# qway/nerfmeshes

Measured on NVIDIA H100. Metric: rays/sec, higher is better.
Workload: dtype f16x3 split operands, f32 accumulate

## Files before the change

include/nerfmeshes_b200.h:

```cpp
#ifndef NERFMESHES_B200_H
#define NERFMESHES_B200_H

#include <stdint.h>

#ifdef __cplusplus
extern "C" {
#endif

#define NM_VERSION 100

typedef struct NmNetDesc {
  int32_t num_layers;
  int32_t hidden_size;
  int32_t skip_step;
  int32_t num_encoding_fn_xyz;
  int32_t num_encoding_fn_dir;
  int32_t include_input_xyz;
  int32_t include_input_dir;
  int32_t log_sampling_xyz;
  int32_t log_sampling_dir;
  int32_t use_viewdirs;
} NmNetDesc;

enum {
// ... 170 lines not shown
int nm_debug_gemm(NmHandle h, const float* a_dev, const float* b_dev, int M, int N, int K, int n_passes, float* d_dev,
                  void* stream);

int nm_debug_mlp_backward(NmHandle h, int which, const float* pts_dev, const float* dirs_dev, int64_t M, const float* dout_dev,
                          void* stream);

int nm_debug_composite_backward(NmHandle h, const float* raw_dev, const float* t_dev, const float* dirs_dev,
                                const float* d_rgb_dev, int64_t R, int S, float noise_std, uint64_t seed, int white_bg,
                                float* dout_dev, void* stream);
int nm_debug_composite(NmHandle h, const float* raw_dev, const float* t_dev, const float* dirs_dev, int64_t R, int S,
                       float noise_std, uint64_t seed, int white_bg, int training, float thr, const NmRenderOut* out_dev,
                       void* stream);
int nm_debug_sample_pdf(NmHandle h, const float* t_c_dev, const float* w_c_dev, const float* u_dev, int64_t R, int Nc, int Nf,
                        int perturb, uint64_t seed, float* t_out_dev, void* stream);

int nm_debug_pack(const NmNetDesc* desc, int n_tensors, const char* const* names, const float* const* tensors_host,
                  const int64_t* numel, int sigma_only, void* program_out, size_t program_cap, uint8_t* pack_out,
                  size_t pack_cap, size_t* pack_need);
int nm_debug_pack_wide(const NmNetDesc* desc, int n_tensors, const char* const* names, const float* const* tensors_host,
                       const int64_t* numel, int sigma_only, void* program_out, size_t program_cap, uint8_t* pack_out,
                       size_t pack_cap, size_t* pack_need);

int nm_debug_tile_schedule(int samples_per_ray, int64_t n_tiles, int grid, int cta, int64_t* tiles_out, int64_t cap, int64_t* n_out);

int nm_kernel_flags(NmHandle h, int32_t* out2);
int nm_check_flags(NmHandle h, void* stream);

int64_t nm_launch_count(NmHandle h);
int nm_set_timing(NmHandle h, int enable);
double nm_mlp_time_ms(NmHandle h, int64_t* points_out, int64_t* launches_out);

#ifdef __cplusplus
}
#endif
#endif
```

nerfmeshes_b200/_lib.py:

```python
import ctypes as C
import os

_HERE = os.path.dirname(os.path.abspath(__file__))
LIB_PATH = os.path.join(_HERE, "lib", "libnerfmeshes_b200.so")


class NmNetDesc(C.Structure):
    _fields_ = [(n, C.c_int32) for n in (
        "num_layers", "hidden_size", "skip_step", "num_encoding_fn_xyz", "num_encoding_fn_dir",
        "include_input_xyz", "include_input_dir", "log_sampling_xyz", "log_sampling_dir", "use_viewdirs")]


class NmRenderCfg(C.Structure):
    _fields_ = [("num_coarse", C.c_int32), ("num_fine", C.c_int32), ("lindisp", C.c_int32), ("perturb", C.c_int32),
                ("white_background", C.c_int32), ("noise_std", C.c_float), ("attenuation_threshold", C.c_float),
                ("precision", C.c_int32), ("act_scale_log2", C.c_int32)]


OUT_FIELDS = ("rgb", "depth", "depth_raw", "acc", "disp", "weights", "mask_weights", "t_vals",
              "coarse_rgb", "coarse_acc", "coarse_disp", "coarse_weights")


class NmRenderOut(C.Structure):
    _fields_ = [(n, C.c_void_p) for n in OUT_FIELDS]
# ... 53 lines not shown
    "nm_query_host": (C.c_int, [_P, _P, _I, _P, _L, _P, _I, C.c_uint64, C.POINTER(NmRenderOut)]),
    "nm_render_image_host": (C.c_int, [_P, _P, _I, _I, _D, _I, _I, _I, _P, _I, C.c_uint64, C.POINTER(NmRenderOut)]),
    "nm_point_mlp_host": (C.c_int, [_P, _I, _P, _P, _L, _P, _I]),
    "nm_zero_grad": (C.c_int, [_P, _P]),
    "nm_backward_rays": (C.c_int, [_P, _P, _I, _P, _L, _P, _P, _P, _I, C.c_uint64, _P, _P, _P]),
    "nm_loss_backward": (C.c_int, [_P, _P, _I, _P, _L, _P, _P, _P, _I, C.c_uint64, _P, _P, _P]),
    "nm_get_grad": (C.c_int, [_P, _I, C.c_char_p, _P, _L, _P]),
    "nm_ray_voxel_indices": (C.c_int, [_P, _P, _I, _P, _L, _P, _P, _P, _P]),
    "nm_ray_voxel_indices_ex": (C.c_int, [_P, _P, _I, _P, _L, _P, _I, C.c_uint64, _P, _P, _P]),
    "nm_tree_integrate": (C.c_int, [_P, _P, _P, _P, _L, _P, C.c_int32, C.c_int32, _P]),
    "nm_debug_gemm": (C.c_int, [_P, _P, _P, _I, _I, _I, _I, _P, _P]),
    "nm_debug_mlp_backward": (C.c_int, [_P, _I, _P, _P, _L, _P, _P]),
    "nm_debug_composite_backward": (C.c_int, [_P, _P, _P, _P, _P, _L, _I, _F, C.c_uint64, _I, _P, _P]),
    "nm_debug_composite": (C.c_int, [_P, _P, _P, _P, _L, _I, _F, C.c_uint64, _I, _I, _F, C.POINTER(NmRenderOut), _P]),
    "nm_debug_sample_pdf": (C.c_int, [_P, _P, _P, _P, _L, _I, _I, _I, C.c_uint64, _P, _P]),
    "nm_debug_pack": (C.c_int, [C.POINTER(NmNetDesc), _I, C.POINTER(C.c_char_p), C.POINTER(_P), C.POINTER(C.c_int64), _I, _P,
                               C.c_size_t, _P, C.c_size_t, C.POINTER(C.c_size_t)]),
    "nm_debug_pack_wide": (C.c_int, [C.POINTER(NmNetDesc), _I, C.POINTER(C.c_char_p), C.POINTER(_P), C.POINTER(C.c_int64), _I,
                                    _P, C.c_size_t, _P, C.c_size_t, C.POINTER(C.c_size_t)]),
    "nm_kernel_flags": (C.c_int, [_P, C.POINTER(C.c_int32)]),
    "nm_check_flags": (C.c_int, [_P, _P]),
    "nm_ndc_rays": (C.c_int, [_P, _I, _I, _D, _D, _P, _I, _P, _L, _P, _P, _P]),
    "nm_launch_count": (C.c_int64, [_P]),
    "nm_debug_tile_schedule": (C.c_int, [_I, _L, _I, _I, _P, _L, _P]),
    "nm_set_timing": (C.c_int, [_P, _I]),
    "nm_mlp_time_ms": (C.c_double, [_P, C.POINTER(C.c_int64), C.POINTER(C.c_int64)]),
}

_lib = None


class NmError(RuntimeError):
    pass


def load():
    global _lib
    if _lib is not None:
        return _lib
    if not os.path.exists(LIB_PATH):
        raise NmError(f"{LIB_PATH} is missing: build it with `python -m nerfmeshes_b200.build` "
                      "(there is no fallback implementation)")
    lib = C.CDLL(LIB_PATH)
    for name, (res, args) in _SIGNATURES.items():
        fn = getattr(lib, name)
        fn.restype = res
        fn.argtypes = args
# ... 12 lines not shown
```

nerfmeshes_b200/csrc/nm_api.cu:

```cuda
#include <cmath>
#include <cstdio>
#include <cstdlib>
#include <algorithm>
#include <cstring>
#include <vector>

#include "nm_common.h"
#include "nm_gemm.h"

namespace nm {
const char* last_error();
}

using namespace nm;

namespace {

struct Buf {
  void* p = nullptr;
  size_t cap = 0;
  int ensure(size_t bytes) {
    if (bytes <= cap) return 0;
    if (p) cudaFree(p);
    p = nullptr; cap = 0;
// ... 9 lines not shown

}

struct NmHandle_t {
  int device = 0;
  int num_sms = 0;
  NmRenderCfg cfg{};
  NetDev nets[2];
  bool has_fine = false;
  NmNetDesc desc[2]{};
  Buf s_table, u_table, voxels;
  int V = 0;
  Buf t_c, raw_c, w_c, t_f, raw_f, t_u, dirs, origins, lin[3], small, stage_in[3], stage_out[12];
  int lin_n[3] = {0, 0, 0};
  int* d_err = nullptr;
  int* h_err = nullptr;
  double* d_stats = nullptr;
  cudaStream_t own_stream = nullptr;
  int64_t launches = 0;
  bool timing = false;
  std::vector<cudaEvent_t> ev;
  size_t ev_used = 0;
  int64_t mlp_points = 0, mlp_launches = 0;
  Buf mc_ws, mc_ws2;
  int64_t mc_counts[2] = {0, 0};
  Buf ss_tab, ss_ws;
  Buf ms_ws, nn_ws;
  Buf cc_ws;
  Buf dc_ws;
  Buf tx_ws;
  Buf rs_ws;
  Buf sf_ws;
  Buf sp_ws;
  int sp_grid[4] = {0, 0, 0, 0};
  const float* sp_vol = nullptr;
  struct OccGrid {
    bool valid = false;
    bool stale = false;
    float lo[3], hi[3], inv[3];
    int G = 0;
    Buf bits;
  } occ[2];
  Buf oc_ws;
  Buf sk_ws;
  Buf ts_ws[2], ts_pts[2];
  Buf train_ws_c;
// ... 95 lines not shown
  }
  return 0;
}

int run_mlp(NmHandle h, int which, bool sigma_only, const MlpInput& in, float* out, cudaStream_t st, const MlpEmit* emit = nullptr,
            const CompositeArgs* comp = nullptr) {
  const NetDev& net = h->nets[which];
  NM_CHECK(net.loaded, "weights of network %d not loaded", which);
  cudaEvent_t e0 = nullptr, e1 = nullptr;
  if (h->timing) {
    while (h->ev.size() < h->ev_used + 2) {
      cudaEvent_t e;
      NM_CUDA(cudaEventCreate(&e));
      h->ev.push_back(e);
    }
    e0 = h->ev[h->ev_used++]; e1 = h->ev[h->ev_used++];
    NM_CUDA(cudaEventRecord(e0, st));
  }
  int rc;
  if (h->cfg.precision == NM_PREC_FP32) rc = launch_mlp_simt(net, sigma_only, in, out, st, &h->launches);
  else rc = launch_mlp_tc(net, sigma_only, h->cfg.precision == NM_PREC_FAST ? 1 : 3, h->cfg.act_scale_log2, in, out,
                          h->num_sms, h->d_err, st, &h->launches, emit, comp);
  if (rc) return rc;
  if (h->timing) {
    NM_CUDA(cudaEventRecord(e1, st));
    h->mlp_points += in.M;
    h->mlp_launches += 1;
  }
  return 0;
}

constexpr uint64_t kNoiseSaltMain = 0x5bd1e995ull, kNoiseSaltCoarse = 0x7f4a7c15a3c59ac3ull;
constexpr uint64_t kVoxelSalt = 0xd1b54a32d192ed03ull, kInvCdfSalt = 0x9e3779b9ull;

struct RayBatch {
  const float* origins; int o_stride; const float* dirs; long long R;
  float nf[2]; const float* near_dev; const float* far_dev;
};

float* off(float* p, long long n) { return p ? p + n : nullptr; }

struct TrainSkip {
  bool emit = false;
  double budget = 0;
  double* committed = nullptr;
  long long M = 0;
// ... 95 lines not shown
    for (long long j0 = 0; j0 < M; j0 += P) {
      const long long m = (M - j0 < P) ? M - j0 : P;
      if (!ts)
        if (int e = launch_occ_stage(idx + j0, m, s, rb.origins, rb.o_stride, rb.dirs, t, pts, dirs, st, &h->launches)) return e;
      MlpInput in{};
      in.mode = IN_POINTS; in.pts = ts ? pts + 3 * j0 : pts; in.dirs = ts ? dirs + 3 * j0 : dirs; in.M = m;
      if (int e = run_mlp(h, which, false, in, out, st, (ts && ts->ws) ? &em : nullptr)) return e;
      if (int e = launch_occ_expand(out, idx + j0, m, raw_buf.as<float>(), st, &h->launches)) return e;
    }
    return 0;
  };
  auto mlp_composite = [&](int which, Buf& raw_buf, const MlpEmit* emit, const float* t, int s, float* rgb, float* depth,
                           float* depth_raw, float* acc, float* disp, float* w, float* mw, uint64_t salt = kNoiseSaltMain) -> int {
    CompositeArgs a{};
    a.t = t; a.dirs = rb.dirs; a.R = R; a.S = s; a.noise_std = c.noise_std; a.seed = seed ^ salt;
    a.white_bg = c.white_background; a.training = training ? 1 : 0; a.thr = c.attenuation_threshold;
    a.rgb = rgb; a.depth = depth; a.depth_raw = depth_raw; a.acc = acc; a.disp = disp; a.weights = w; a.mask_weights = mw;
    if (skip || tsk) {
      if (int e = skip_raw(which, raw_buf, t, s, tsk ? &tsk[which] : nullptr)) return e;
      a.raw = raw_buf.as<float>();
      return launch_composite(a, st, &h->launches);
    }
    const bool fuse = fused_env && !need_raw && !emit && c.precision != NM_PREC_FP32 && mlp_tc_composite_group(s) > 0;
    if (fuse) return run_mlp(h, which, false, rays_input(t, s), nullptr, st, nullptr, &a);
    if (int e = raw_buf.ensure((size_t)R * s * 16)) return e;
    if (int e = run_mlp(h, which, false, rays_input(t, s), raw_buf.as<float>(), st, emit)) return e;
    a.raw = raw_buf.as<float>();
    return launch_composite(a, st, &h->launches);
  };

  if (teacher) {
    NM_CHECK(o.t_vals != nullptr, "NM_FLAG_TEACHER_T needs out.t_vals as input");
    const int which = (h->has_fine && !buff) ? NM_NET_FINE : NM_NET_COARSE;
    return mlp_composite(which, h->raw_f, nullptr, o.t_vals, S, o.rgb, o.depth, o.depth_raw, o.acc, o.disp, o.weights, o.mask_weights);
  }

  if (int e = h->t_c.ensure((size_t)R * Nc * 4)) return e;
  float* t_c = h->t_c.as<float>();
  if (int e = launch_stratified(h->s_table.as<float>(), Nc, R, rb.nf, rb.near_dev, rb.far_dev, c.lindisp, c.perturb,
                                seed, t_c, st, &h->launches)) return e;
  if (buff) {
    NM_CHECK(h->V > 0, "BuFF render without a voxel list (nm_set_tree)");
    NM_CHECK(rb.near_dev == nullptr, "BuFF path takes scalar near/far");
    if (int e = h->t_u.ensure((size_t)R * Nc * 4)) return e;
    float* z = h->t_u.as<float>();
    if (int e = launch_aabb(h->voxels.as<float>(), h->V, rb.origins, rb.o_stride, rb.dirs, R, rb.nf[0], rb.nf[1], Nc,
                            h->s_table.as<float>(), t_c, z, nullptr, h->d_err + 1, st, &h->launches,
// ... 1122 lines not shown
  if (int e = bind_device(h)) return e;
  NM_CUDA(cudaStreamSynchronize((cudaStream_t)stream));
  return check_kernel_flags(h);
}

int nm_ndc_rays(NmHandle h, int H, int W, double focal, double near, const float* origins_dev, int o_stride,
                const float* dirs_dev, int64_t n, float* origins_out_dev, float* dirs_out_dev, void* stream) {
  if (int e = bind_device(h)) return e;
  NM_CHECK(origins_dev && dirs_dev && origins_out_dev && dirs_out_dev && n >= 0, "bad arguments");
  NM_CHECK(o_stride == 0 || o_stride == 3, "o_stride must be 0 or 3");
  return launch_ndc(H, W, focal, near, origins_dev, o_stride, dirs_dev, n, origins_out_dev, dirs_out_dev, (cudaStream_t)stream,
                    &h->launches);
}

int nm_kernel_flags(NmHandle h, int32_t* out2) {
  NM_CHECK(h && out2, "null argument");
  out2[0] = h->h_err[0];
  out2[1] = h->h_err[1];
  return 0;
}

int64_t nm_launch_count(NmHandle h) { return h ? h->launches : -1; }

int nm_debug_tile_schedule(int samples_per_ray, int64_t n_tiles, int grid, int cta, int64_t* tiles_out, int64_t cap, int64_t* n_out) {
  const int g = mlp_tc_composite_group(samples_per_ray);
  if (tiles_out && n_out) {
    const int64_t gt = g > 0 ? g : 1;
    int64_t n = 0;
    for (int64_t i = 0;; ++i) {
      const int64_t grp = cta + (i / gt) * grid, t = grp * gt + (i % gt);
      if (t >= n_tiles) break;
      if (n < cap) tiles_out[n] = t;
      ++n;
    }
    *n_out = n;
  }
  return g;
}

int nm_set_timing(NmHandle h, int enable) {
  NM_CHECK(h, "null handle");
  h->timing = enable != 0;
  h->ev_used = 0; h->mlp_points = 0; h->mlp_launches = 0;
  return 0;
}

double nm_mlp_time_ms(NmHandle h, int64_t* points_out, int64_t* launches_out) {
  if (!h || !h->timing) return -1.0;
  cudaSetDevice(h->device);
  double total = 0.0;
  for (size_t i = 0; i + 1 < h->ev_used; i += 2) {
    if (cudaEventSynchronize(h->ev[i + 1]) != cudaSuccess) return -1.0;
    float ms = 0.f;
    if (cudaEventElapsedTime(&ms, h->ev[i], h->ev[i + 1]) != cudaSuccess) return -1.0;
    total += ms;
  }
  if (points_out) *points_out = h->mlp_points;
  if (launches_out) *launches_out = h->mlp_launches;
  h->ev_used = 0; h->mlp_points = 0; h->mlp_launches = 0;
  return total;
// ... 108 lines not shown
```

nerfmeshes_b200/csrc/nm_common.h:

```cpp
#pragma once
#include <cuda_runtime.h>
#include <stdint.h>

#include <functional>
#include <string>
#include <vector>

#include "../../include/nerfmeshes_b200.h"
#include "nm_program.h"

namespace nm {

void set_error(const char* fmt, ...);
#define NM_CUDA(expr)                                                                             \
  do {                                                                                            \
    cudaError_t _e = (expr);                                                                      \
    if (_e != cudaSuccess) {                                                                      \
      nm::set_error("%s failed: %s (%s:%d)", #expr, cudaGetErrorString(_e), __FILE__, __LINE__); \
      return -2;                                                                                  \
    }                                                                                             \
  } while (0)
#define NM_CHECK(cond, ...)       \
  do {                            \
    if (!(cond)) {                \
// ... 62 lines not shown
  uint32_t* bits[kMaxLayers];
  float* act[kMaxLayers];
  int kbt;
};

int build_programs(const NmNetDesc& d, NetProgram* full, NetProgram* sigma);
int build_backward_program(const NetProgram& full, NetProgram* bwd);
int build_backward_stream(NetDev* net, cudaStream_t st, int64_t* launches);
struct WeightSource {
  int n = 0;
  const char* const* names = nullptr;
  const float* const* ptrs = nullptr;
  const int64_t* numel = nullptr;
  const float* find(const std::string& name, int64_t expect) const;
};
int pack_network(const NmNetDesc& d, const WeightSource& src, NetDev* net);
int load_network_dev(const NmNetDesc& d, const WeightSource& src_device, NetDev* net, cudaStream_t st, int64_t* launches);
void free_network(NetDev* net);
int debug_pack(const NmNetDesc& d, const WeightSource& src, bool sigma_only, bool wide, NetProgram* prog, uint8_t* out,
               size_t cap, size_t* need);

struct CompositeArgs;
int mlp_tc_composite_group(int samples_per_ray);
int launch_mlp_tc(const NetDev& net, bool sigma_only, int n_passes, int act_scale_log2, const MlpInput& in, float* out,
                  int num_sms, int* d_err, cudaStream_t st, int64_t* launches, const MlpEmit* emit = nullptr,
                  const CompositeArgs* comp = nullptr);
int launch_mlp_tc_bwd(const NetDev& net, long long M, const float* dz_in, int dz_ld, const float* dout,
                      const MlpEmit& io, int n_passes, int num_sms, int* d_err, cudaStream_t st, int64_t* launches);
int launch_mlp_simt(const NetDev& net, bool sigma_only, const MlpInput& in, float* out, cudaStream_t st,
                    int64_t* launches);

struct RayGenArgs {
  float pose[12];
  int H, W;
  double focal;
  int ndc;
  double ndc_near;
  int row0, row1;
};
int launch_raygen(const RayGenArgs& a, float* origins_or_null, float* dirs, cudaStream_t st, int64_t* launches);
int launch_ndc(int H, int W, double focal, double near, const float* origins, int o_stride, const float* dirs, long long n,
               float* out_o, float* out_d, cudaStream_t st, int64_t* launches);
int launch_stratified(const float* s_table, int Nc, long long R, const float* near_far2, const float* near_dev,
                      const float* far_dev, int lindisp, int perturb, uint64_t seed, float* t_out, cudaStream_t st,
                      int64_t* launches);
struct CompositeArgs {
// ... 198 lines not shown
```

nerfmeshes_b200/csrc/nm_mlp_tc.cu:

```cuda
#include <cuda_bf16.h>
#include <cuda_fp16.h>

#include <cstdio>
#include <cstdlib>
#include <vector>

#include "nm_common.h"
#include "nm_composite.cuh"
#include "nm_frontend.cuh"
#include "nm_ptx.cuh"

namespace nm {

namespace {

constexpr int kThreads = 384;
constexpr int kProdWarp = 8;
constexpr uint32_t kKBlock = 2 * 8192;
constexpr uint32_t kActBytes = 4 * kKBlock;
constexpr uint32_t kWgBytes = kActBytes + kKBlock;
constexpr int kMaxStages = 8;
constexpr uint32_t kCompBytes = 64 * 16 + 64 * 4 + 64 * 4 + 64;

struct TcParams {
  NetProgram net;
  const uint8_t* wpack;
  const float* bias;
  const float* head;
  MlpInput in;
  float* out;
  int out_sigma_only;
  int n_passes;
  float act_scale, act_inv_scale;
  int num_stages;
  long long n_tiles;
  int* err;
  uint32_t off_wg, off_bias, off_head, off_bars, off_comp;
  int has_emit;
  MlpEmit emit;
  int mode;
  const float* dz_in;
  int dz_ld;
  const float* dout;
  int comp_on;
  int tile_group;
  CompositeArgs comp;
};
static_assert(sizeof(TcParams) <= 4096, "TcParams must fit the 4 KB kernel-parameter window");

#ifndef NM_MLP_STALLS
#define NM_MLP_STALLS 0
#endif
#if NM_MLP_STALLS
#define NM_ST(...) __VA_ARGS__
#else
#define NM_ST(...)
#endif

constexpr uint32_t kBarWFull = 0, kBarWEmpty = 128, kBarStalls = 192, kBarBytes = 192 + (NM_MLP_STALLS ? 128 : 0);

// ... 25 lines not shown
#pragma unroll
  for (int k = 0; k < 4; ++k)
    if (HH) ptx::wgmma<W, 0, 0, BF16>(d, a_hi + 2 * k, b_hi + 2 * k, 1u);
#pragma unroll
  for (int k = 0; k < 4; ++k)
    if (LH) ptx::wgmma<W, 0, 0, BF16>(d, a_lo + 2 * k, b_hi + 2 * k, 1u);
#pragma unroll
  for (int k = 0; k < 4; ++k)
    if (HL) ptx::wgmma<W, 0, 0, BF16>(d, a_hi + 2 * k, b_lo + 2 * k, 1u);
}

template <int V>
struct IntC {
  static constexpr int value = V;
};

template <int MODE>
__global__ void __launch_bounds__(kThreads, 1) mlp_tc_kernel(const __grid_constant__ TcParams P) {
  extern __shared__ __align__(1024) uint8_t smem[];
  const uint32_t sbase = ptx::smem_u32(smem);
  const int warp = __shfl_sync(0xffffffffu, (int)(threadIdx.x >> 5), 0), lane = threadIdx.x & 31;
  const uint32_t bars = sbase + P.off_bars;
  const int NS = P.num_stages;
  float* s_bias = reinterpret_cast<float*>(smem + P.off_bias);
  float* s_head = reinterpret_cast<float*>(smem + P.off_head);
  const int n_layers = P.net.n_layers;

  if (threadIdx.x == 0) {
    if (sbase & 1023u) { atomicExch(P.err, ERR_ALIGN); __trap(); }
    for (int i = 0; i < kMaxStages; ++i) {
      ptx::mbar_init(bars + kBarWFull + 8 * i, 1);
      ptx::mbar_init(bars + kBarWFull + 64 + 8 * i, 1);
      ptx::mbar_init(bars + kBarWEmpty + 8 * i, 1);
    }
    ptx::fence_mbar_init();
  }
  for (int i = threadIdx.x; i < P.net.n_bias; i += kThreads) s_bias[i] = (MODE == 2) ? 0.f : P.bias[i];
  for (int i = threadIdx.x; i < P.net.n_head; i += kThreads) s_head[i] = P.head[i];
  __syncthreads();

  const uint32_t Gt = (uint32_t)P.tile_group, V = 2u * gridDim.x, v0 = 2u * blockIdx.x;
  auto tile_of = [&](uint32_t v, uint32_t i) -> long long {
    const long long g = (long long)v + (long long)(i / Gt) * (long long)V;
    const long long t = g * (long long)Gt + (long long)(i % Gt);
    return t < P.n_tiles ? t : -1;
  };

  if (warp >= kProdWarp) {
    asm volatile("setmaxnreg.dec.sync.aligned.u32 40;");
    if (warp == kProdWarp && lane == 0) {
      int slot = 0;
      uint32_t ph = 0;
      const bool exact = P.n_passes == 3;
      for (uint32_t i = 0; tile_of(v0, i) >= 0; ++i) {
        const int n_wg = tile_of(v0 + 1, i) >= 0 ? 2 : 1;
        int b0 = 0;
        for (int li = 0; li < n_layers; ++li) {
          const LayerProg& L = P.net.layers[li];
          const bool wide = wide_width(L) == 128;
          const uint32_t bytes = (exact || wide) ? (uint32_t)kStageBytes : (uint32_t)kHalfStage;
          const int b1 = b0 + wide_stages(L);
// ... 41 lines not shown
      float p[3], d[3];
      fetch_point(P.in, m, p, d);
      auto emit = [&](int j, float val) {
        const float a = val * si;
        const uint16_t h = f16_bits_sat(a);
        const uint32_t off = swz_off(t, j);
        *reinterpret_cast<uint16_t*>(pe + off) = h;
        *reinterpret_cast<uint16_t*>(pe + 8192 + off) = f16_bits_sat(a - f16_bits_to_float(h));
      };
      const int dim = dir ? P.net.dim_dir : P.net.dim_xyz;
      for (int j = dim; j < 64; ++j) {
        const uint32_t off = swz_off(t, j);
        *reinterpret_cast<uint16_t*>(pe + off) = 0;
        *reinterpret_cast<uint16_t*>(pe + 8192 + off) = 0;
      }
      if (dir) positional_encoding(d, Ld, idr, P.net.freq_dir, emit);
      else positional_encoding(p, Lx, ix, P.net.freq_xyz, emit);
    }
    ptx::fence_proxy_async_smem();
    ptx::named_bar_sync(bar_id, 128);
    NM_ST(if (t == 0) st[3] += clock64() - c0;)
  };

  uint8_t* comp_s = smem + P.off_comp + (uint32_t)wg * kCompBytes;
  auto composite_tile = [&](uint32_t itp, long long tp) {
    const CompositeArgs& A = P.comp;
    const int r = t;
    float4* stage = reinterpret_cast<float4*>(comp_s);
    float* keepT = reinterpret_cast<float*>(comp_s + 64 * 16);
    float* wv = keepT + 64;
    const float* carry_in = wv + 64 + ((itp & 1) ^ 1) * 8;
    float* carry_out = wv + 64 + (itp & 1) * 8;
    const long long p0 = tp * kTileM, p1 = min(p0 + (long long)kTileM, P.in.M);
    const int S = A.S;
    const long long ray_first = p0 / S;
    const int n_seg = (int)((p1 - 1) / S - ray_first) + 1;
    ptx::named_bar_sync(bar_id, 128);
    const long long p = p0 + r;
    const bool live = r < kTileM && p < p1;
    float tc = 0.f, alpha = 0.f;
    float4 q = make_float4(0.f, 0.f, 0.f, 0.f);
    if (live) {
      const long long ray = p / S;
      const int i = (int)(p - ray * S);
      const float* tr = A.t + ray * S;
      tc = tr[i];
      const float tn = (i + 1 < S) ? tr[i + 1] : 0.f;
      q = stage[r];
      float keep;
      alpha = comp_alpha(A, ray, i, tc, tn, comp_ray_norm(A.dirs, ray), q.w, &keep);
      keepT[r] = keep;
    }
    ptx::named_bar_sync(bar_id, 128);
    for (int k = r; k < n_seg; k += 128) {
      const long long rayk = ray_first + k;
// ... 144 lines not shown
      if (writes_a) ptx::named_bar_sync(bar_id, 128);
      auto chunks = [&](auto plain) {
        constexpr bool PLAIN = decltype(plain)::value;
        const int heads_c = PLAIN ? 0 : heads;
        const bool writes_c = PLAIN || writes_a;
#pragma unroll
        for (int nc = 0; nc < 4; ++nc) {
          if (nc >= NC) continue;
          uint32_t mk_in[2][2] = {{0xffffffffu, 0xffffffffu}, {0xffffffffu, 0xffffffffu}};
          if (MODE == 2 && L.kind == KIND_BWD && L.relu) {
#pragma unroll
            for (int e = 0; e < 2; ++e) {
              const long long m = e ? m1 : m0;
              if (e ? val1 : val0) {
                const uint2 bw = *reinterpret_cast<const uint2*>(P.emit.bits[li] + (size_t)m * (size_t)(L.n_out >> 5) + (size_t)(nc * 2));
                mk_in[e][0] = bw.x; mk_in[e][1] = bw.y;
              }
            }
          }
          uint32_t mk_out[2][2] = {{0u, 0u}, {0u, 0u}};
#pragma unroll
          for (int j8 = 0; j8 < 8; ++j8) {
            const int col = nc * 64 + j8 * 8 + cq;
            float x[2][2];
#pragma unroll
            for (int e = 0; e < 2; ++e) {
              const bool valid = e ? val1 : val0;
              const long long m = e ? m1 : m0;
              if (MODE == 2 && L.kind == KIND_LOAD) {
                const float2 z = valid ? *reinterpret_cast<const float2*>(P.dz_in + (size_t)m * P.dz_ld + col) : make_float2(0.f, 0.f);
                x[e][0] = z.x; x[e][1] = z.y;
              } else if (MODE == 2) {
#pragma unroll
                for (int u = 0; u < 2; ++u) {
                  float y = acc[nc * 32 + j8 * 4 + 2 * e + u] * so;
                  if (L.aux2) y = fmaf(dsg[e], s_head[L.head_off + col + u], y);
                  const uint32_t w = valid ? mk_in[e][j8 >> 2] : 0u;
                  x[e][u] = ((w >> ((col + u) & 31)) & 1u) ? y : 0.f;
                }
              } else {
#pragma unroll
                for (int u = 0; u < 2; ++u) {
                  float y = fmaf(acc[nc * 32 + j8 * 4 + 2 * e + u], so, s_bias[L.bias_off + col + u]);
                  if (L.relu) y = fmaxf(y, 0.f);
                  x[e][u] = y;
                }
              }
            }
#pragma unroll
            for (int hh = 0; hh < 4; ++hh) {
              if (hh >= heads_c) break;
              const float* w = s_head + L.head_off + hh * L.n_out + col;
#pragma unroll
              for (int e = 0; e < 2; ++e) {
                part[e][hh] = fmaf(w[0], x[e][0], part[e][hh]);
                part[e][hh] = fmaf(w[1], x[e][1], part[e][hh]);
              }
            }
#pragma unroll
            for (int e = 0; e < 2; ++e) {
              const bool valid = e ? val1 : val0;
              const long long m = e ? m1 : m0;
              const int row = r0 + 8 * e;
              if (MODE == 1) {
                mk_out[e][j8 >> 2] |= ((x[e][0] > 0.f ? 1u : 0u) | (x[e][1] > 0.f ? 2u : 0u)) << (col & 31);
                if (P.emit.act[li] && valid) *reinterpret_cast<float2*>(P.emit.act[li] + (size_t)m * L.n_out + col) = make_float2(x[e][0], x[e][1]);
              }
              if (writes_c) {
                uint32_t hi, lo;
                const float a0 = x[e][0] * si, a1 = x[e][1] * si;
                if (MODE == 2) {
                  split_bf16x2(a0, a1, &hi, &lo);
                } else {
                  hi = ptx::pack_f16x2_sat(a0, a1);
                  const float2 f = __half22float2(*reinterpret_cast<const __half2*>(&hi));
                  lo = ptx::pack_f16x2_sat(a0 - f.x, a1 - f.y);
                }
                if (n_passes != 3) lo = 0u;
                const uint32_t off = (uint32_t)nc * kKBlock + swz_off(row, col & 63);
// ... 30 lines not shown
                const long long m = e ? m1 : m0;
                if ((lane & 3) == 0 && (e ? val1 : val0)) P.emit.bits[li][(size_t)m * (size_t)(L.n_out >> 5) + (size_t)(nc * 2 + g)] = w;
              }
          }
        }
      };
      if constexpr (MODE == 0) {
        if (heads == 0 && writes_a) chunks(IntC<1>{}); else chunks(IntC<0>{});
      } else {
        chunks(IntC<0>{});
      }
      if (writes_a) {
        ptx::fence_proxy_async_smem();
        ptx::named_bar_sync(bar_id, 128);
      }
      if (heads) {
#pragma unroll
        for (int e = 0; e < 2; ++e)
#pragma unroll
          for (int hh = 0; hh < 4; ++hh) {
            part[e][hh] += __shfl_xor_sync(0xffffffffu, part[e][hh], 1);
            part[e][hh] += __shfl_xor_sync(0xffffffffu, part[e][hh], 2);
          }
        const float* hb = s_head + L.head_off + heads * L.n_out;
#pragma unroll
        for (int e = 0; e < 2; ++e) {
          const long long m = e ? m1 : m0;
          const bool valid = e ? val1 : val0;
          if (L.kind == KIND_SIGMA) {
            sigma_val[e] = part[e][0] + hb[0];
            if (L.is_final && (lane & 3) == 0 && valid && P.out) P.out[m] = sigma_val[e];
          } else if ((lane & 3) == 0 && (P.comp_on || (valid && P.out))) {
            float o[4];
#pragma unroll
            for (int hh = 0; hh < 4; ++hh) o[hh] = (hh < heads) ? part[e][hh] + hb[hh] : 0.f;
            const float sg = (L.kind == KIND_RGB) ? sigma_val[e] : o[3];
            if (P.out_sigma_only) {
              P.out[m] = sg;
            } else {
              float4 res;
              res.x = 1.f / (1.f + expf(-o[0]));
              res.y = 1.f / (1.f + expf(-o[1]));
              res.z = 1.f / (1.f + expf(-o[2]));
              res.w = sg;
              if (MODE == 0 && P.comp_on) reinterpret_cast<float4*>(comp_s)[r0 + 8 * e] = res;
              else reinterpret_cast<float4*>(P.out)[m] = res;
            }
          }
        }
      }
      NM_ST(if (t == 0) st[4] += clock64() - ce;)
    }
    if (MODE == 0 && P.comp_on) {
      NM_ST(const long long c0 = clock64();)
      composite_tile(it, tile);
      NM_ST(if (t == 0) st[5] += clock64() - c0;)
    }
  }
  NM_ST(if (t == 0 && (blockIdx.x < 2 || blockIdx.x + 1 == gridDim.x))
          printf("mlp_stalls mode %d cta %d wg %d wait %lld mma %lld encode %lld epilogue %lld composite %lld other %lld\n", MODE,
                 (int)blockIdx.x, wg, st[0], st[1], st[3], st[4], st[5], clock64() - st[2] - st[0] - st[1] - st[3] - st[4] - st[5]);)
}

}

static int launch_prepared(TcParams& P, int num_sms, cudaStream_t st, int64_t* launches) {
  const NetProgram& hp = P.net;
  {
    bool dir_seen = false;
    for (int i = 0; i < hp.n_layers; ++i) {
      NM_CHECK(!(dir_seen && hp.layers[i].pe_src == SRC_PE_XYZ), "xyz encoding read after the view-direction encoding");
      if (hp.layers[i].pe_src == SRC_PE_DIR) dir_seen = true;
    }
  }
  auto align_up = [](uint32_t x, uint32_t a) { return (x + a - 1) / a * a; };
  int dev = 0, max_smem = 0;
  NM_CUDA(cudaGetDevice(&dev));
  NM_CUDA(cudaDeviceGetAttribute(&max_smem, cudaDevAttrMaxSharedMemoryPerBlockOptin, dev));
  const uint32_t fixed = 2 * kWgBytes + align_up(hp.n_bias * 4, 16) + align_up((hp.n_head > 0 ? hp.n_head : 4) * 4, 16) +
                         kBarBytes + (P.comp_on ? 2 * kCompBytes : 0u);
  int ns = ((int)max_smem - (int)fixed) / kStageBytes;
  if (ns > kMaxStages) ns = kMaxStages;
  NM_CHECK(ns >= 2, "network too large for the shared-memory budget (%u B fixed, %d B available)", fixed, max_smem);
  P.num_stages = ns;
  for (int i = 0; i < hp.n_layers; ++i)
    NM_CHECK(hp.layers[i].kind == KIND_LOAD || hp.layers[i].n_out == 64 || hp.layers[i].n_out == 128 || hp.layers[i].n_out == 256,
             "layer %d: output width %d not 64, 128 or 256", i, hp.layers[i].n_out);
  uint32_t off = (uint32_t)ns * kStageBytes;
  P.off_wg = off; off += 2 * kWgBytes;
  P.off_bias = off; off += align_up(hp.n_bias * 4, 16);
  P.off_head = off; off += align_up((hp.n_head > 0 ? hp.n_head : 4) * 4, 16);
  P.off_bars = off; off += kBarBytes;
  P.off_comp = off; off += P.comp_on ? 2 * kCompBytes : 0u;
  if (P.tile_group < 1) P.tile_group = 1;
  NM_CHECK((int)off <= max_smem, "shared-memory layout overflow");

  const int mode = P.mode == 2 ? 2 : (P.has_emit ? 1 : 0);
  auto kern = mode == 2 ? mlp_tc_kernel<2> : (mode == 1 ? mlp_tc_kernel<1> : mlp_tc_kernel<0>);
  static thread_local unsigned configured_devs[3] = {0, 0, 0};
  if (!(configured_devs[mode] & (1u << (dev & 31)))) {
    NM_CUDA(cudaFuncSetAttribute(kern, cudaFuncAttributeMaxDynamicSharedMemorySize, max_smem));
    configured_devs[mode] |= 1u << (dev & 31);
  }
  const long long n_groups = (P.n_tiles + P.tile_group - 1) / P.tile_group;
  const long long pairs = (n_groups + 1) / 2;
  const long long grid = pairs < num_sms ? pairs : num_sms;
  kern<<<(unsigned)grid, kThreads, off, st>>>(P);
  NM_CUDA(cudaGetLastError());
  if (launches) ++*launches;
  return 0;
}

int mlp_tc_composite_group(int S) {
  if (S <= 0) return 0;
  int a = S, b = kTileM;
  while (b) { const int t = a % b; a = b; b = t; }
  const long long l = (long long)S / a * kTileM;
  const long long g = l / kTileM;
  return g <= 16 ? (int)g : 0;
}
// ... 1 lines not shown
int launch_mlp_tc(const NetDev& net, bool sigma_only, int n_passes, int act_scale_log2, const MlpInput& in, float* out,
                  int num_sms, int* d_err, cudaStream_t st, int64_t* launches, const MlpEmit* emit, const CompositeArgs* comp) {
  if (in.M <= 0) return 0;
  const NetProgram& hp = sigma_only ? net.sigma : net.full;
  TcParams P{};
  P.net = hp;
  P.wpack = sigma_only ? net.d_wpack_sigma : net.d_wpack_full;
  P.bias = net.d_bias;
  P.head = net.d_head;
  P.in = in;
  P.out = out;
  P.out_sigma_only = sigma_only ? 1 : 0;
  P.n_passes = n_passes;
  P.act_scale = ldexpf(1.f, act_scale_log2);
  P.act_inv_scale = ldexpf(1.f, -act_scale_log2);
  P.n_tiles = (in.M + kTileM - 1) / kTileM;
  P.err = d_err;
  if (emit) {
    P.has_emit = 1; P.emit = *emit;
    P.n_tiles = 2 * ((in.M + 127) / 128);
  }
  P.tile_group = 1;
  if (comp) {
    NM_CHECK(!emit && !sigma_only && in.mode == IN_RAYS && comp->S == in.S && comp->R * (long long)comp->S == in.M && comp->t == in.t,
             "fused compositor: needs the ray front end on the compositor's own samples");
    P.tile_group = mlp_tc_composite_group(comp->S);
    NM_CHECK(P.tile_group > 0, "fused compositor: %d samples per ray not supported", comp->S);
    P.comp_on = 1; P.comp = *comp; P.out = nullptr;
  }
  return launch_prepared(P, num_sms, st, launches);
}

int launch_mlp_tc_bwd(const NetDev& net, long long M, const float* dz_in, int dz_ld, const float* dout,
                      const MlpEmit& io, int n_passes, int num_sms, int* d_err, cudaStream_t st, int64_t* launches) {
  if (M <= 0) return 0;
  NM_CHECK(net.bwd_valid && net.d_wpack_bwd, "backward weight stream not built");
  NM_CHECK((dz_ld & 1) == 0 && (reinterpret_cast<uintptr_t>(dz_in) & 7) == 0, "dz_in must be 8-byte aligned rows");
  TcParams P{};
  P.net = net.bwd;
  P.wpack = net.d_wpack_bwd;
  P.bias = net.d_bias;
  P.head = net.d_head;
  P.in.M = M;
  P.n_passes = n_passes;
  P.act_scale = 1.f; P.act_inv_scale = 1.f;
  P.n_tiles = 2 * ((M + 127) / 128);
  P.err = d_err;
  P.has_emit = 1; P.emit = io;
  P.mode = 2; P.dz_in = dz_in; P.dz_ld = dz_ld; P.dout = dout;
  return launch_prepared(P, num_sms, st, launches);
// ... 4 lines not shown
```

nerfmeshes_b200/engine.py:

```python
from __future__ import annotations

import ctypes as C
from dataclasses import dataclass
from typing import Dict, Optional

import numpy as np
import torch

from . import _lib as L

NET_KEYS = ("num_layers", "hidden_size", "skip_step", "num_encoding_fn_xyz", "num_encoding_fn_dir",
            "include_input_xyz", "include_input_dir", "log_sampling_xyz", "log_sampling_dir", "use_viewdirs")
NET_DEFAULTS = dict(num_layers=4, hidden_size=128, skip_step=4, num_encoding_fn_xyz=6, num_encoding_fn_dir=4,
                    include_input_xyz=True, include_input_dir=True, log_sampling_xyz=True, log_sampling_dir=True,
                    use_viewdirs=True)


def net_desc(**kw) -> L.NmNetDesc:
    d = dict(NET_DEFAULTS)
    d.update({k: v for k, v in kw.items() if k in NET_KEYS})
    return L.NmNetDesc(*[int(d[k]) for k in NET_KEYS])


@dataclass
# ... 702 lines not shown
        from .mesh import clamp_iso_level
        mn, mx, sd = self.sparse_lattice(lins, block, out)
        iso = float(clamp_iso_level(iso_level, np.float32(mn), np.float32(mx), np.float32(sd)))
        return iso, self.sparse_run(lins, block, iso, out)

    def debug_sparse_state(self, shape, block):
        n0, n1, n2 = shape
        W = (n2 + 31) // 32
        nb = [(n - 1 + block - 1) // block for n in shape]
        words = torch.empty((n0, n1, W), dtype=torch.int32, device=self.device)
        state = torch.empty(nb, dtype=torch.int32, device=self.device)
        L.check(self.lib.nm_debug_sparse_sweep_state(self._h, _ptr(words), _ptr(state), self._stream()))
        bits = (words[..., None] >> torch.arange(32, device=self.device, dtype=torch.int32)) & 1
        return bits.reshape(n0, n1, W * 32)[..., :n2].bool(), state

    def kernel_flags(self):
        out = (C.c_int32 * 2)()
        L.check(self.lib.nm_kernel_flags(self._h, out))
        return int(out[0]), int(out[1])

    def launch_count(self) -> int:
        return int(self.lib.nm_launch_count(self._h))

    def set_timing(self, on: bool):
        L.check(self.lib.nm_set_timing(self._h, int(on)))

    def mlp_time_ms(self):
        pts, n = C.c_int64(0), C.c_int64(0)
        ms = float(self.lib.nm_mlp_time_ms(self._h, C.byref(pts), C.byref(n)))
        return ms, int(pts.value), int(n.value)
```

Before: 654,600.

## Run coarse pass sigma-only in fused compositor and free bias/head shared memory

In inference with a fine pass, the coarse network now runs the sigma-only program inside the fused compositor, because the coarse colour is not needed. This skips the view-direction and RGB layers for coarse samples. For the inference kernel mode, bias and head weights are read through __ldg from global memory instead of being staged in shared memory. The compositor staging buffer now reuses the positional-encoding scratch, with only a small carry area kept, so more shared memory is left for extra pipeline stages. The risks are extra global loads in the epilogue, a new named barrier before the final write, and correctness depending on the sigma-only gating conditions.

```diff
diff --git a/include/nerfmeshes_b200.h b/include/nerfmeshes_b200.h
--- a/include/nerfmeshes_b200.h
+++ b/include/nerfmeshes_b200.h
@@ -216,11 +216,14 @@
                        size_t pack_cap, size_t* pack_need);
 
 int nm_debug_tile_schedule(int samples_per_ray, int64_t n_tiles, int grid, int cta, int64_t* tiles_out, int64_t cap, int64_t* n_out);
+int nm_debug_mlp_layout(const void* program, size_t program_size, int max_smem, int comp_on, int training, int slot_cap,
+                        int64_t* out5);
 
 int nm_kernel_flags(NmHandle h, int32_t* out2);
 int nm_check_flags(NmHandle h, void* stream);
 
 int64_t nm_launch_count(NmHandle h);
+int64_t nm_sigma_only_points(NmHandle h);
 int nm_set_timing(NmHandle h, int enable);
 double nm_mlp_time_ms(NmHandle h, int64_t* points_out, int64_t* launches_out);
 
diff --git a/nerfmeshes_b200/_lib.py b/nerfmeshes_b200/_lib.py
--- a/nerfmeshes_b200/_lib.py
+++ b/nerfmeshes_b200/_lib.py
@@ -99,7 +99,9 @@
     "nm_check_flags": (C.c_int, [_P, _P]),
     "nm_ndc_rays": (C.c_int, [_P, _I, _I, _D, _D, _P, _I, _P, _L, _P, _P, _P]),
     "nm_launch_count": (C.c_int64, [_P]),
+    "nm_sigma_only_points": (C.c_int64, [_P]),
     "nm_debug_tile_schedule": (C.c_int, [_I, _L, _I, _I, _P, _L, _P]),
+    "nm_debug_mlp_layout": (C.c_int, [_P, C.c_size_t, _I, _I, _I, _I, _P]),
     "nm_set_timing": (C.c_int, [_P, _I]),
     "nm_mlp_time_ms": (C.c_double, [_P, C.POINTER(C.c_int64), C.POINTER(C.c_int64)]),
 }
diff --git a/nerfmeshes_b200/csrc/nm_api.cu b/nerfmeshes_b200/csrc/nm_api.cu
--- a/nerfmeshes_b200/csrc/nm_api.cu
+++ b/nerfmeshes_b200/csrc/nm_api.cu
@@ -55,6 +55,7 @@
   std::vector<cudaEvent_t> ev;
   size_t ev_used = 0;
   int64_t mlp_points = 0, mlp_launches = 0;
+  int64_t sigma_points = 0;
   Buf mc_ws, mc_ws2;
   int64_t mc_counts[2] = {0, 0};
   Buf ss_tab, ss_ws;
@@ -196,6 +197,7 @@
   else rc = launch_mlp_tc(net, sigma_only, h->cfg.precision == NM_PREC_FAST ? 1 : 3, h->cfg.act_scale_log2, in, out,
                           h->num_sms, h->d_err, st, &h->launches, emit, comp);
   if (rc) return rc;
+  if (sigma_only) h->sigma_points += in.M;
   if (h->timing) {
     NM_CUDA(cudaEventRecord(e1, st));
     h->mlp_points += in.M;
@@ -337,7 +339,10 @@
       return launch_composite(a, st, &h->launches);
     }
     const bool fuse = fused_env && !need_raw && !emit && c.precision != NM_PREC_FP32 && mlp_tc_composite_group(s) > 0;
-    if (fuse) return run_mlp(h, which, false, rays_input(t, s), nullptr, st, nullptr, &a);
+    const NetProgram& sp = h->nets[which].sigma;
+    const bool sigma_only = fuse && which == NM_NET_COARSE && Nf > 0 && !training && rgb == nullptr &&
+                            sp.layers[sp.n_layers - 1].kind == KIND_SIGMA;
+    if (fuse) return run_mlp(h, which, sigma_only, rays_input(t, s), nullptr, st, nullptr, &a);
     if (int e = raw_buf.ensure((size_t)R * s * 16)) return e;
     if (int e = run_mlp(h, which, false, rays_input(t, s), raw_buf.as<float>(), st, emit)) return e;
     a.raw = raw_buf.as<float>();
@@ -1506,6 +1511,8 @@
 
 int64_t nm_launch_count(NmHandle h) { return h ? h->launches : -1; }
 
+int64_t nm_sigma_only_points(NmHandle h) { return h ? h->sigma_points : -1; }
+
 int nm_debug_tile_schedule(int samples_per_ray, int64_t n_tiles, int grid, int cta, int64_t* tiles_out, int64_t cap, int64_t* n_out) {
   const int g = mlp_tc_composite_group(samples_per_ray);
   if (tiles_out && n_out) {
@@ -1520,6 +1527,17 @@
     *n_out = n;
   }
   return g;
+}
+
+int nm_debug_mlp_layout(const void* program, size_t program_size, int max_smem, int comp_on, int training, int slot_cap,
+                        int64_t* out5) {
+  NM_CHECK(program && out5, "null argument");
+  NM_CHECK(program_size >= sizeof(NetProgram), "program buffer too small (%zu needed)", sizeof(NetProgram));
+  MlpTcLayout l;
+  if (int e = mlp_tc_layout(*reinterpret_cast<const NetProgram*>(program), max_smem, comp_on != 0, training != 0, slot_cap, &l)) return e;
+  const int64_t v[5] = {l.num_stages, l.off_wg, l.off_bars, l.off_carry, l.bytes};
+  for (int i = 0; i < 5; ++i) out5[i] = v[i];
+  return 0;
 }
 
 int nm_set_timing(NmHandle h, int enable) {
diff --git a/nerfmeshes_b200/csrc/nm_common.h b/nerfmeshes_b200/csrc/nm_common.h
--- a/nerfmeshes_b200/csrc/nm_common.h
+++ b/nerfmeshes_b200/csrc/nm_common.h
@@ -108,6 +108,11 @@
 
 struct CompositeArgs;
 int mlp_tc_composite_group(int samples_per_ray);
+struct MlpTcLayout {
+  int num_stages;
+  uint32_t off_wg, off_bias, off_head, off_bars, off_carry, bytes;
+};
+int mlp_tc_layout(const NetProgram& prog, int max_smem, bool comp_on, bool training, int slot_cap, MlpTcLayout* out);
 int launch_mlp_tc(const NetDev& net, bool sigma_only, int n_passes, int act_scale_log2, const MlpInput& in, float* out,
                   int num_sms, int* d_err, cudaStream_t st, int64_t* launches, const MlpEmit* emit = nullptr,
                   const CompositeArgs* comp = nullptr);
diff --git a/nerfmeshes_b200/csrc/nm_mlp_tc.cu b/nerfmeshes_b200/csrc/nm_mlp_tc.cu
--- a/nerfmeshes_b200/csrc/nm_mlp_tc.cu
+++ b/nerfmeshes_b200/csrc/nm_mlp_tc.cu
@@ -20,7 +20,7 @@
 constexpr uint32_t kActBytes = 4 * kKBlock;
 constexpr uint32_t kWgBytes = kActBytes + kKBlock;
 constexpr int kMaxStages = 8;
-constexpr uint32_t kCompBytes = 64 * 16 + 64 * 4 + 64 * 4 + 64;
+constexpr uint32_t kCarryBytes = 64;
 
 struct TcParams {
   NetProgram net;
@@ -35,7 +35,7 @@
   int num_stages;
   long long n_tiles;
   int* err;
-  uint32_t off_wg, off_bias, off_head, off_bars, off_comp;
+  uint32_t off_wg, off_bias, off_head, off_bars, off_carry;
   int has_emit;
   MlpEmit emit;
   int mode;
@@ -107,9 +107,12 @@
   const int warp = __shfl_sync(0xffffffffu, (int)(threadIdx.x >> 5), 0), lane = threadIdx.x & 31;
   const uint32_t bars = sbase + P.off_bars;
   const int NS = P.num_stages;
+  const int n_layers = P.net.n_layers;
   float* s_bias = reinterpret_cast<float*>(smem + P.off_bias);
   float* s_head = reinterpret_cast<float*>(smem + P.off_head);
-  const int n_layers = P.net.n_layers;
+  const float* vbias = MODE == 0 ? P.bias : s_bias;
+  const float* vhead = MODE == 0 ? P.head : s_head;
+  auto ldv = [](const float* p) -> float { if constexpr (MODE == 0) return __ldg(p); else return *p; };
 
   if (threadIdx.x == 0) {
     if (sbase & 1023u) { atomicExch(P.err, ERR_ALIGN); __trap(); }
@@ -120,8 +123,10 @@
     }
     ptx::fence_mbar_init();
   }
-  for (int i = threadIdx.x; i < P.net.n_bias; i += kThreads) s_bias[i] = (MODE == 2) ? 0.f : P.bias[i];
-  for (int i = threadIdx.x; i < P.net.n_head; i += kThreads) s_head[i] = P.head[i];
+  if (MODE != 0) {
+    for (int i = threadIdx.x; i < P.net.n_bias; i += kThreads) s_bias[i] = (MODE == 2) ? 0.f : P.bias[i];
+    for (int i = threadIdx.x; i < P.net.n_head; i += kThreads) s_head[i] = P.head[i];
+  }
   __syncthreads();
 
   const uint32_t Gt = (uint32_t)P.tile_group, V = 2u * gridDim.x, v0 = 2u * blockIdx.x;
@@ -209,15 +214,15 @@
     NM_ST(if (t == 0) st[3] += clock64() - c0;)
   };
 
-  uint8_t* comp_s = smem + P.off_comp + (uint32_t)wg * kCompBytes;
+  float* carry = reinterpret_cast<float*>(smem + P.off_carry + (uint32_t)wg * kCarryBytes);
   auto composite_tile = [&](uint32_t itp, long long tp) {
     const CompositeArgs& A = P.comp;
     const int r = t;
-    float4* stage = reinterpret_cast<float4*>(comp_s);
-    float* keepT = reinterpret_cast<float*>(comp_s + 64 * 16);
+    float4* stage = reinterpret_cast<float4*>(pe);
+    float* keepT = reinterpret_cast<float*>(pe + 64 * 16);
     float* wv = keepT + 64;
-    const float* carry_in = wv + 64 + ((itp & 1) ^ 1) * 8;
-    float* carry_out = wv + 64 + (itp & 1) * 8;
+    const float* carry_in = carry + ((itp & 1) ^ 1) * 8;
+    float* carry_out = carry + (itp & 1) * 8;
     const long long p0 = tp * kTileM, p1 = min(p0 + (long long)kTileM, P.in.M);
     const int S = A.S;
     const long long ray_first = p0 / S;
@@ -408,6 +413,9 @@
 #pragma unroll
           for (int j8 = 0; j8 < 8; ++j8) {
             const int col = nc * 64 + j8 * 8 + cq;
+            float2 bias2 = make_float2(0.f, 0.f);
+            if constexpr (MODE == 0) bias2 = __ldg(reinterpret_cast<const float2*>(vbias + L.bias_off + col));
+            else if constexpr (MODE == 1) bias2 = *reinterpret_cast<const float2*>(vbias + L.bias_off + col);
             float x[2][2];
 #pragma unroll
             for (int e = 0; e < 2; ++e) {
@@ -420,14 +428,14 @@
 #pragma unroll
                 for (int u = 0; u < 2; ++u) {
                   float y = acc[nc * 32 + j8 * 4 + 2 * e + u] * so;
-                  if (L.aux2) y = fmaf(dsg[e], s_head[L.head_off + col + u], y);
+                  if (L.aux2) y = fmaf(dsg[e], ldv(vhead + L.head_off + col + u), y);
                   const uint32_t w = valid ? mk_in[e][j8 >> 2] : 0u;
                   x[e][u] = ((w >> ((col + u) & 31)) & 1u) ? y : 0.f;
                 }
               } else {
 #pragma unroll
                 for (int u = 0; u < 2; ++u) {
-                  float y = fmaf(acc[nc * 32 + j8 * 4 + 2 * e + u], so, s_bias[L.bias_off + col + u]);
+                  float y = fmaf(acc[nc * 32 + j8 * 4 + 2 * e + u], so, u ? bias2.y : bias2.x);
                   if (L.relu) y = fmaxf(y, 0.f);
                   x[e][u] = y;
                 }
@@ -436,11 +444,12 @@
 #pragma unroll
             for (int hh = 0; hh < 4; ++hh) {
               if (hh >= heads_c) break;
-              const float* w = s_head + L.head_off + hh * L.n_out + col;
+              const float* w = vhead + L.head_off + hh * L.n_out + col;
+              const float w0 = ldv(w), w1 = ldv(w + 1);
 #pragma unroll
               for (int e = 0; e < 2; ++e) {
-                part[e][hh] = fmaf(w[0], x[e][0], part[e][hh]);
-                part[e][hh] = fmaf(w[1], x[e][1], part[e][hh]);
+                part[e][hh] = fmaf(w0, x[e][0], part[e][hh]);
+                part[e][hh] = fmaf(w1, x[e][1], part[e][hh]);
               }
             }
 #pragma unroll
@@ -517,18 +526,22 @@
             part[e][hh] += __shfl_xor_sync(0xffffffffu, part[e][hh], 1);
             part[e][hh] += __shfl_xor_sync(0xffffffffu, part[e][hh], 2);
           }
-        const float* hb = s_head + L.head_off + heads * L.n_out;
+        const float* hb = vhead + L.head_off + heads * L.n_out;
+        if (MODE == 0 && P.comp_on && L.is_final) ptx::named_bar_sync(bar_id, 128);
 #pragma unroll
         for (int e = 0; e < 2; ++e) {
           const long long m = e ? m1 : m0;
           const bool valid = e ? val1 : val0;
           if (L.kind == KIND_SIGMA) {
-            sigma_val[e] = part[e][0] + hb[0];
-            if (L.is_final && (lane & 3) == 0 && valid && P.out) P.out[m] = sigma_val[e];
+            sigma_val[e] = part[e][0] + ldv(hb);
+            if (L.is_final && (lane & 3) == 0) {
+              if (MODE == 0 && P.comp_on) reinterpret_cast<float4*>(pe)[r0 + 8 * e] = make_float4(0.f, 0.f, 0.f, sigma_val[e]);
+              else if (valid && P.out) P.out[m] = sigma_val[e];
+            }
           } else if ((lane & 3) == 0 && (P.comp_on || (valid && P.out))) {
             float o[4];
 #pragma unroll
-            for (int hh = 0; hh < 4; ++hh) o[hh] = (hh < heads) ? part[e][hh] + hb[hh] : 0.f;
+            for (int hh = 0; hh < 4; ++hh) o[hh] = (hh < heads) ? part[e][hh] + ldv(hb + hh) : 0.f;
             const float sg = (L.kind == KIND_RGB) ? sigma_val[e] : o[3];
             if (P.out_sigma_only) {
               P.out[m] = sg;
@@ -538,7 +551,7 @@
               res.y = 1.f / (1.f + expf(-o[1]));
               res.z = 1.f / (1.f + expf(-o[2]));
               res.w = sg;
-              if (MODE == 0 && P.comp_on) reinterpret_cast<float4*>(comp_s)[r0 + 8 * e] = res;
+              if (MODE == 0 && P.comp_on) reinterpret_cast<float4*>(pe)[r0 + 8 * e] = res;
               else reinterpret_cast<float4*>(P.out)[m] = res;
             }
           }
@@ -557,6 +570,36 @@
                  (int)blockIdx.x, wg, st[0], st[1], st[3], st[4], st[5], clock64() - st[2] - st[0] - st[1] - st[3] - st[4] - st[5]);)
 }
 
+}
+
+int mlp_tc_layout(const NetProgram& hp, int max_smem, bool comp_on, bool training, int slot_cap, MlpTcLayout* out) {
+  auto align_up = [](uint32_t x, uint32_t a) { return (x + a - 1) / a * a; };
+  const uint32_t vb = training ? align_up(hp.n_bias * 4, 16) : 0u, vh = training ? align_up((hp.n_head > 0 ? hp.n_head : 4) * 4, 16) : 0u;
+  const uint32_t fixed = 2 * kWgBytes + vb + vh + kBarBytes + (comp_on ? 2 * kCarryBytes : 0u);
+  int ns = ((int)max_smem - (int)fixed) / (int)kStageBytes;
+  NM_CHECK(ns >= 2, "network too large for the shared-memory budget (%u B fixed, %d B available)", fixed, max_smem);
+  if (ns > kMaxStages) ns = kMaxStages;
+  if (slot_cap > 0 && ns > slot_cap) ns = slot_cap < 2 ? 2 : slot_cap;
+  for (int i = 0; i < hp.n_layers; ++i)
+    NM_CHECK(hp.layers[i].kind == KIND_LOAD || hp.layers[i].n_out == 64 || hp.layers[i].n_out == 128 || hp.layers[i].n_out == 256,
+             "layer %d: output width %d not 64, 128 or 256", i, hp.layers[i].n_out);
+  MlpTcLayout l{};
+  l.num_stages = ns;
+  uint32_t off = (uint32_t)ns * kStageBytes;
+  l.off_wg = off; off += 2 * kWgBytes;
+  l.off_bias = off; off += vb;
+  l.off_head = off; off += vh;
+  l.off_bars = off; off += kBarBytes;
+  l.off_carry = off; off += comp_on ? 2 * kCarryBytes : 0u;
+  l.bytes = off;
+  NM_CHECK((int)off <= max_smem, "shared-memory layout overflow");
+  *out = l;
+  return 0;
+}
+
+static int ring_slot_cap() {
+  const char* e = getenv("NM_MLP_RING_SLOTS");
+  return e ? atoi(e) : 0;
 }
 
 static int launch_prepared(TcParams& P, int num_sms, cudaStream_t st, int64_t* launches) {
@@ -568,29 +611,17 @@
       if (hp.layers[i].pe_src == SRC_PE_DIR) dir_seen = true;
     }
   }
-  auto align_up = [](uint32_t x, uint32_t a) { return (x + a - 1) / a * a; };
   int dev = 0, max_smem = 0;
   NM_CUDA(cudaGetDevice(&dev));
   NM_CUDA(cudaDeviceGetAttribute(&max_smem, cudaDevAttrMaxSharedMemoryPerBlockOptin, dev));
-  const uint32_t fixed = 2 * kWgBytes + align_up(hp.n_bias * 4, 16) + align_up((hp.n_head > 0 ? hp.n_head : 4) * 4, 16) +
-                         kBarBytes + (P.comp_on ? 2 * kCompBytes : 0u);
-  int ns = ((int)max_smem - (int)fixed) / kStageBytes;
-  if (ns > kMaxStages) ns = kMaxStages;
-  NM_CHECK(ns >= 2, "network too large for the shared-memory budget (%u B fixed, %d B available)", fixed, max_smem);
-  P.num_stages = ns;
-  for (int i = 0; i < hp.n_layers; ++i)
-    NM_CHECK(hp.layers[i].kind == KIND_LOAD || hp.layers[i].n_out == 64 || hp.layers[i].n_out == 128 || hp.layers[i].n_out == 256,
-             "layer %d: output width %d not 64, 128 or 256", i, hp.layers[i].n_out);
-  uint32_t off = (uint32_t)ns * kStageBytes;
-  P.off_wg = off; off += 2 * kWgBytes;
-  P.off_bias = off; off += align_up(hp.n_bias * 4, 16);
-  P.off_head = off; off += align_up((hp.n_head > 0 ? hp.n_head : 4) * 4, 16);
-  P.off_bars = off; off += kBarBytes;
-  P.off_comp = off; off += P.comp_on ? 2 * kCompBytes : 0u;
+  const int mode = P.mode == 2 ? 2 : (P.has_emit ? 1 : 0);
+  MlpTcLayout lay;
+  if (int e = mlp_tc_layout(hp, max_smem, P.comp_on != 0, mode != 0, ring_slot_cap(), &lay)) return e;
+  P.num_stages = lay.num_stages;
+  P.off_wg = lay.off_wg; P.off_bias = lay.off_bias; P.off_head = lay.off_head; P.off_bars = lay.off_bars; P.off_carry = lay.off_carry;
+  const uint32_t off = lay.bytes;
   if (P.tile_group < 1) P.tile_group = 1;
-  NM_CHECK((int)off <= max_smem, "shared-memory layout overflow");
-
-  const int mode = P.mode == 2 ? 2 : (P.has_emit ? 1 : 0);
+
   auto kern = mode == 2 ? mlp_tc_kernel<2> : (mode == 1 ? mlp_tc_kernel<1> : mlp_tc_kernel<0>);
   static thread_local unsigned configured_devs[3] = {0, 0, 0};
   if (!(configured_devs[mode] & (1u << (dev & 31)))) {
@@ -638,10 +669,12 @@
   }
   P.tile_group = 1;
   if (comp) {
-    NM_CHECK(!emit && !sigma_only && in.mode == IN_RAYS && comp->S == in.S && comp->R * (long long)comp->S == in.M && comp->t == in.t,
+    NM_CHECK(!emit && in.mode == IN_RAYS && comp->S == in.S && comp->R * (long long)comp->S == in.M && comp->t == in.t,
              "fused compositor: needs the ray front end on the compositor's own samples");
     P.tile_group = mlp_tc_composite_group(comp->S);
     NM_CHECK(P.tile_group > 0, "fused compositor: %d samples per ray not supported", comp->S);
+    NM_CHECK(!sigma_only || (!comp->rgb && hp.layers[hp.n_layers - 1].kind == KIND_SIGMA),
+             "fused compositor: the sigma-only program must end in a sigma layer and write no colour map");
     P.comp_on = 1; P.comp = *comp; P.out = nullptr;
   }
   return launch_prepared(P, num_sms, st, launches);
diff --git a/nerfmeshes_b200/engine.py b/nerfmeshes_b200/engine.py
--- a/nerfmeshes_b200/engine.py
+++ b/nerfmeshes_b200/engine.py
@@ -748,6 +748,9 @@
     def launch_count(self) -> int:
         return int(self.lib.nm_launch_count(self._h))
 
+    def sigma_only_points(self) -> int:
+        return int(self.lib.nm_sigma_only_points(self._h))
+
     def set_timing(self, on: bool):
         L.check(self.lib.nm_set_timing(self._h, int(on)))
 
```

After: 722,200, median of 6. 10.3% higher.
